# chennachaos/PFEMFort

Measured on AMD Instinct MI355X. Metric: DOF/s (assembly+CG-to-tol), higher is better.
Workload: dtype f64

## Files before the change

### include/pfem_amd_diag.h

```cpp
#ifndef PFEM_AMD_DIAG_H
#define PFEM_AMD_DIAG_H

#include "pfem_amd.h"

#ifdef __cplusplus
extern "C" {
#endif

#define PFEM_ASSEMBLY_GATHER 0
#define PFEM_ASSEMBLY_SCATTER 1
int pfem_solver_set_assembly_mode(pfem_solver *s, int mode);
int pfem_solver_assembly_info(pfem_solver *s, int *gather_form, int *hub_nodes, int *block_threads, int64_t *lds_bytes);
#define PFEM_SPMV_AUTO 0
#define PFEM_SPMV_INT32 1
#define PFEM_SPMV_GAPS16 2
#define PFEM_SPMV_GROUPED 3
int pfem_solver_set_spmv_format(pfem_solver *s, int format);
int pfem_solver_get_spmv_format(pfem_solver *s, int *bits_per_column);
int pfem_solver_get_spmv_row_group(pfem_solver *s, int *rows_per_lane);
int pfem_solver_get_spmv_gap_table(pfem_solver *s, int *entries);
int pfem_solver_get_spmv_value_dictionary(pfem_solver *s, int *entries);
int pfem_solver_amg_value_dictionaries(pfem_solver *s, int max_levels, int *n_levels, int *entries);
int pfem_solver_get_spmv_gap_escapes(pfem_solver *s, int *in_use);
int pfem_solver_spmv_bytes(pfem_solver *s, int64_t *format_bytes);

int pfem_solver_amg_info(pfem_solver *s, int max_levels, int *n_levels, int64_t *rows, int64_t *nnz, double *lambda_max,
                         double *symbolic_ms, double *numeric_ms, int *cheb_degree, int *fine_degree, double *eig_ratio, double *coarse_scale);
int pfem_solver_amg_aggregates(pfem_solver *s, int level, int32_t *agg);
int pfem_solver_amg_transfer(pfem_solver *s, int level, int *rbm, int *fine_bs, int *coarse_bs, int *dim, int64_t *n_nodes, double *node_xyz);
int pfem_solver_amg_layout(pfem_solver *s, int max_levels, int *coupled, int *distributed_levels, int64_t *first_dof, int64_t *local_rows);
int pfem_solver_incidence_patterns(pfem_solver *s, int *count, int *longest);
int pfem_solver_amg_aggregation(pfem_solver *s, int max_levels, int *n_levels, int *kind);
int pfem_solver_amg_comm_counts(pfem_solver *s, int *exchanges_per_cycle, int *allreduces_per_cycle);
int pfem_solver_amg_cycle_profile(pfem_solver *s, int max_levels, int *n_levels, int *exchanges, double *exchange_ms,
                                  int64_t *exchange_doubles, int *allreduces, double *allreduce_ms, int64_t *allreduce_doubles,
                                  double *cycle_ms);
int pfem_solver_amg_pairing(pfem_solver *s, int *lattice_levels);
int pfem_solver_amg_cycle(pfem_solver *s, int *cycle, int *last_level_visited_twice);
int pfem_solver_amg_level0_epilogue(pfem_solver *s, int *taken);

int pfem_eval_elems(pfem_solver *s, const double *elemData, const double *timeData,
                    double *K_out, double *F_out);

int pfem_matrix_info(pfem_solver *s, int64_t *n_owned, int64_t *n_local, int64_t *nnz,
                     int64_t *stored_entries);

int pfem_spmv(pfem_solver *s, const double *x, double *y);
int pfem_bench_spmv(pfem_solver *s, int reps, double *ms_per_launch);

typedef struct pfem_timings {
    double pattern_ms;
    double assemble_ms;
    double solve_ms;
    double spmv_ms_total;
    int64_t spmv_launches;
// ... 28 lines not shown
```

### pfemfort_amd/_lib.py

```python
from __future__ import annotations

import ctypes as C
import os

_HERE = os.path.dirname(os.path.abspath(__file__))
LIB_PATH = os.environ.get("PFEM_AMD_LIB") or os.path.join(_HERE, "libpfem_amd.so")

OK, ERR_ARG, ERR_STATE, ERR_NEG_JAC, ERR_HIP, ERR_NOGPU, ERR_NOMEM, ERR_DIVERGED, ERR_PATTERN, ERR_COMM = range(10)
POISSON_TRIA, POISSON_TET, ELAST_TET, POISSON_TRIA_INLINE, ELAST_TRIA = 1, 2, 3, 4, 5
SOLVER_EMPTY, PATTERN_OK, INIT_OK, ASSEMBLY_OK, FACTORISE_OK = 1, 2, 3, 4, 5
INSERT_VALUES, ADD_VALUES = 1, 2

NPELEM = {POISSON_TRIA: 3, POISSON_TET: 4, ELAST_TET: 4, POISSON_TRIA_INLINE: 3, ELAST_TRIA: 3}
NDOF = {POISSON_TRIA: 1, POISSON_TET: 1, ELAST_TET: 3, POISSON_TRIA_INLINE: 1, ELAST_TRIA: 2}
NDIM = {POISSON_TRIA: 2, POISSON_TET: 3, ELAST_TET: 3, POISSON_TRIA_INLINE: 2, ELAST_TRIA: 2}


class PfemError(RuntimeError):
    def __init__(self, code: int, where: str, detail: str = ""):
        self.code = code
        msg = f"{where}: error {code} ({_strerror(code)})"
        if detail:
            msg += f" -- {detail}"
        super().__init__(msg)
# ... 40 lines not shown
    "pfem_write_vtk": [C.c_char_p, _I, _L, _L, _I, _I, _P, _P, _P, _P],
    "pfem_write_temp_dat": [C.c_char_p, _L, _P, _P, _P],
    "pfem_solver_create": [_P, _L, _L, _L, _P, _P, _I],
    "pfem_solver_destroy": [_P],
    "pfem_solver_set_stream": [_P, _P],
    "pfem_solver_set_tolerances": [_P, _D, _D, _D, _I],
    "pfem_solver_status": [_P, _P],
    "pfem_solver_set_zero": [_P],
    "pfem_solver_print_info": [_P],
    "pfem_mat_set_values": [_P, _I, _P, _I, _P, _P, _I],
    "pfem_vec_set_values": [_P, _I, _P, _P, _I],
    "pfem_solver_assemble_matrix_and_vector": [_P, _I, _P, _P, _P, _P],
    "pfem_solver_factorise": [_P],
    "pfem_solver_solve": [_P, _P, _P, _P],
    "pfem_solver_factorise_and_solve": [_P, _P, _P, _P],
    "pfem_solver_get_solution": [_P, _P],
    "pfem_solver_get_history": [_P, _P, _I, _P],
    "pfem_mesh_upload": [_P, _I, _L, _P, _L, _P, _P, _P],
    "pfem_box_slab_sizes": [_I, _I, _I, _I, _I, _I, _I, _P, _P, _P, _P, _P],
    "pfem_mesh_generate_box": [_P, _I, _D, _D, _I, _D, _D, _I, _D, _D, _I, _I, _I, _I],
    "pfem_box_slab_sizes_axis": [_I, _I, _I, _I, _I, _I, _I, _I, _P, _P, _P, _P, _P, _P, _P, _P],
    "pfem_mesh_generate_box_axis": [_P, _I, _D, _D, _I, _D, _D, _I, _D, _D, _I, _I, _I, _I, _I],
    "pfem_mesh_download": [_P, _P, _P, _P, _P],
    "pfem_pattern_build": [_P],
    "pfem_assemble": [_P, _P, _P],
    "pfem_solver_set_assembly_mode": [_P, _I],
    "pfem_solver_assembly_info": [_P, _P, _P, _P, _P],
    "pfem_solver_set_spmv_format": [_P, _I],
    "pfem_solver_get_spmv_format": [_P, _P],
    "pfem_solver_get_spmv_row_group": [_P, _P],
    "pfem_solver_get_spmv_gap_table": [_P, _P],
    "pfem_solver_get_spmv_value_dictionary": [_P, _P],
    "pfem_solver_amg_value_dictionaries": [_P, _I, _P, _P],
    "pfem_solver_get_spmv_gap_escapes": [_P, _P],
    "pfem_solver_spmv_bytes": [_P, _P],
    "pfem_solver_set_preconditioner": [_P, _I],
    "pfem_solver_get_preconditioner": [_P, _P],
    "pfem_solver_set_cg_single_reduction": [_P, _I],
    "pfem_solver_amg_info": [_P, _I, _P, _P, _P, _P, _P, _P, _P, _P, _P, _P],
    "pfem_solver_amg_aggregates": [_P, _I, _P],
    "pfem_solver_amg_transfer": [_P, _I, _P, _P, _P, _P, _P, _P],
    "pfem_solver_amg_layout": [_P, _I, _P, _P, _P, _P],
    "pfem_solver_amg_aggregation": [_P, _I, _P, _P],
    "pfem_solver_incidence_patterns": [_P, _P, _P],
    "pfem_solver_amg_comm_counts": [_P, _P, _P],
    "pfem_solver_amg_cycle_profile": [_P, _I, _P, _P, _P, _P, _P, _P, _P, _P],
    "pfem_solver_amg_pairing": [_P, _P],
    "pfem_solver_set_amg_options": [_P, _I, _I, _D, _D],
    "pfem_solver_set_amg_cycle": [_P, _I],
    "pfem_solver_amg_cycle": [_P, _P, _P],
    "pfem_solver_amg_level0_epilogue": [_P, _P],
    "pfem_eval_elems": [_P, _P, _P, _P, _P],
    "pfem_rhs_add_values": [_P, _L, _P, _P],
    "pfem_matrix_info": [_P, _P, _P, _P, _P],
    "pfem_get_local_to_global": [_P, _P],
    "pfem_get_csr": [_P, _P, _P, _P],
    "pfem_get_rhs": [_P, _P],
    "pfem_spmv": [_P, _P, _P],
    "pfem_bench_spmv": [_P, _I, _P],
    "pfem_get_timings": [_P, _P],
    "pfem_solver_profile_spmv": [_P, _I],
    "pfem_neighbour_plan": [_I, _I, _P, _P, _P, _P, _P, _P, _P, _P, _P],
    "pfem_solver_set_neighbours": [_P, _I, _P, _P, _P],
    "pfem_rccl_unique_id": [_P],
    "pfem_solver_set_comm_rccl": [_P, _I, _I, _P],
    "pfem_solver_set_comm_host": [_P, _I, _I, HOST_ALLREDUCE_FN, HOST_EXCHANGE_FN, _P],
# ... 61 lines not shown
```

### pfemfort_amd/csrc/pfem_amg.inc

```

constexpr int kAmgMaxLevels = 14;
constexpr int kAmgMatchRounds = 8;
constexpr int kAmgPasses = 3;
constexpr int64_t kAmgReplicateRows = 150000;
constexpr int kAmgRetryBlock = -7701;

inline bool amg_in_effect(const pfem_solver *s)
{
    return s->pc == PFEM_PC_GAMG;
}

inline SellDev amg_sell(const pfem_solver *s, const AmgLevel &L, int64_t rows)
{
    SellDev A;
    if (L.fine) {
        A = s->sell();
    } else {
        A.slice_off = L.slice_off.p;
        A.rowlen = L.rowlen.p;
        A.cols = L.cols.p;
        A.vals = L.vals.p;
    }
    A.n_rows = rows;
    A.n_slices = (rows + 63) / 64;
// ... 2162 lines not shown
                uint64_t last = 0;
                PFEM_HIP(hipMemcpyAsync(&last, ukeys.p + (nnz_c - 1), sizeof(uint64_t), hipMemcpyDeviceToHost, s->stream));
                PFEM_HIP(hipStreamSynchronize(s->stream));
                if (last == ~0ull) --nnz_c;
            }
            L.nnz_c = nnz_c;
            PFEM_TRY(amg_sell_from_keys(s, W, ukeys.p, nnz_c, C));
            PFEM_TRY(L.dst_slot.alloc(static_cast<size_t>(std::max<int64_t>(nnz_c, 1))));
            hipLaunchKernelGGL(k_amg_dst_slots, dim3(grid_for(nnz_c)), dim3(kBlock), 0, s->stream, nnz_c, static_cast<const uint64_t *>(ukeys.p),
                               static_cast<const int64_t *>(C.rowptr.p), static_cast<const int64_t *>(C.slice_off.p), L.dst_slot.p);
            PFEM_TRY(check_kernel("k_amg_dst_slots"));
            PFEM_HIP(hipStreamSynchronize(s->stream));
        }
        phase(l, "Galerkin maps + coarse pattern");
        if (coupled) PFEM_TRY(amg_agree(s, C.stored > INT_MAX ? PFEM_ERR_ARG : PFEM_OK));
        else if (C.stored > INT_MAX) return PFEM_ERR_ARG;
        M.lev.push_back(std::move(Cp));
        {
            AmgLevel &Cn = *M.lev.back();
            amg_galerkin(s, L, Cn, A);
            PFEM_TRY(check_kernel("k_amg_galerkin (symbolic)"));
        }
        n_global = nc_global;
        if (coupled && n_global > kAmgDense && n_global <= static_cast<double>(replicate_rows)) {
            PFEM_TRY(amg_replicate(s, M, W, *M.lev.back(), static_cast<int64_t>(n_global), overlap));
            phase(l, "replicated levels");
            break;
        }
    }
    M.n_last_global = coupled ? static_cast<int64_t>(n_global) : M.lev.back()->n;
    return PFEM_OK;
}

int amg_finish_levels(pfem_solver *s, Amg &M, bool coupled)
{
    for (auto &L : M.lev) PFEM_TRY(amg_alloc_vectors(s, *L));
    AmgLevel &last = *M.lev.back();
    const int64_t n_last = M.n_last_global;
    M.dense = n_last >= 1 && n_last <= kAmgDense && M.lev.size() > 1 && !M.rep;
    if (M.dense) {
        PFEM_TRY(M.dense_inv.alloc(static_cast<size_t>(n_last * n_last)));
        const int bytes = static_cast<int>(n_last * n_last * sizeof(double));
        if (bytes > 65536) {
            PFEM_HIP(hipFuncSetAttribute(reinterpret_cast<const void *>(k_amg_dense_inverse), hipFuncAttributeMaxDynamicSharedMemorySize, bytes));
            PFEM_HIP(hipFuncSetAttribute(reinterpret_cast<const void *>(k_amg_dense_inverse_of), hipFuncAttributeMaxDynamicSharedMemorySize, bytes));
        }
        if (coupled) {
            PFEM_TRY(M.dense_glob.alloc(static_cast<size_t>(n_last * n_last)));
            PFEM_TRY(M.bx_glob.alloc(static_cast<size_t>(2 * kAmgDense)));
            PFEM_TRY(amg_level_gids(s, last));
        }
    }
    if (coupled) PFEM_TRY(M.lam_all.alloc(static_cast<size_t>(std::max<int64_t>(256, 2 * static_cast<int64_t>(M.lev.size()) * s->nranks))));
    M.fused = !coupled && [] { const char *e = std::getenv("PFEM_AMG_FUSED"); return e ? std::atoi(e) != 0 : true; }();
    M.tail_from = -1;
    for (size_t l = 1; l < M.lev.size() && !coupled; ++l)
        if (M.lev[l]->n <= kAmgTailRows && M.lev[l]->nnz <= kAmgTailNnz && M.lev.size() - l <= static_cast<size_t>(kAmgTailLevels)) { M.tail_from = static_cast<int>(l); break; }
    M.w_to = M.tail_from > 0 ? M.tail_from : static_cast<int>(M.lev.size()) - 2;
    M.tail_lds_allowed = 0;
    if (M.tail_from > 0) {
        int64_t rows = 0;
        for (size_t l = static_cast<size_t>(M.tail_from); l < M.lev.size(); ++l) rows += M.lev[l]->n;
        const AmgLevel &T0 = *M.lev[static_cast<size_t>(M.tail_from)];
        const size_t need = static_cast<size_t>(6 * rows) * sizeof(double) + static_cast<size_t>(T0.stored) * 12 + static_cast<size_t>((T0.n + 63) / 64 + 2) * 8;
        if (need > 65536 && need <= 156 * 1024) {
            if (hipFuncSetAttribute(reinterpret_cast<const void *>(k_amg_tail), hipFuncAttributeMaxDynamicSharedMemorySize, static_cast<int>(need)) == hipSuccess)
                M.tail_lds_allowed = need;
            else
                (void)hipGetLastError();
        }
    }
    return PFEM_OK;
}


void amg_knobs(Amg &M)
{
    const char *er = std::getenv("PFEM_AMG_EIG_RATIO"), *cs = std::getenv("PFEM_AMG_COARSE_SCALE");
    M.eig_ratio = er ? std::max(1.5, std::atof(er)) : (M.eig_ratio_given ? M.eig_ratio_opt : M.eig_ratio_auto);
    M.coarse_scale = cs ? std::atof(cs) : (M.coarse_scale_given ? M.coarse_scale_opt : M.coarse_scale_auto);
    if (M.rep) { M.rep->eig_ratio = M.eig_ratio; M.rep->coarse_scale = M.coarse_scale; }
}

int amg_symbolic(pfem_solver *s, bool multi, bool overlap)
{
    if (!s->amg) s->amg.reset(new (std::nothrow) Amg());
    if (!s->amg) return PFEM_ERR_NOMEM;
    Amg &M = *s->amg;
    const auto t0 = std::chrono::steady_clock::now();
    const bool verbose = std::getenv("PFEM_AMG_VERBOSE") != nullptr;
    const size_t malloc_calls0 = dev_pool().st_malloc_calls;
    const size_t malloc_bytes0 = dev_pool().st_malloc;
    const double malloc_ms0 = dev_pool().st_malloc_ms;
    const size_t reused0 = dev_pool().st_reused;
    auto since_t0 = [&](const char *what) {
        if (!verbose) return;
        (void)hipStreamSynchronize(s->stream);
        std::fprintf(stderr, "  gamg symbolic: %-40s at %9.2f ms\n", what, std::chrono::duration<double, std::milli>(std::chrono::steady_clock::now() - t0).count());
    };
    M.coupled = multi && !M.coupled_refused && [] { const char *e = std::getenv("PFEM_AMG_COUPLED"); return e ? std::atoi(e) != 0 : true; }();
    const bool coupled = M.coupled;
    if (const char *e = std::getenv("PFEM_AMG_CHEB_DEGREE")) M.cheb_degree = std::max(1, std::min(6, std::atoi(e)));
    if (const char *e = std::getenv("PFEM_AMG_FINE_DEGREE")) M.fine_degree = std::max(0, std::min(6, std::atoi(e)));
    M.lev.clear();
    M.rep.reset();
// ... 530 lines not shown
        if (L.rbm) {
            PFEM_RBM_DISPATCH(L.bs, L.dim, hipLaunchKernelGGL((k_rbm_prolong<FB, DIM>), dim3(vec_grid(L.n_loc / L.bs)), dim3(kBlock), 0, s->stream, L.n_loc / L.bs,
                static_cast<const int32_t *>(L.node_agg.p), static_cast<const double *>(L.roff.p), L.n_loc / L.bs, static_cast<const double *>(C.x),
                M.coarse_scale, L.x, ctl));
        } else
        hipLaunchKernelGGL(k_amg_prolong, dim3(vec_grid(L.n_loc)), dim3(kBlock), 0, s->stream, L.n_loc, static_cast<const int32_t *>(L.agg.p),
                           static_cast<const double *>(C.x), M.coarse_scale, L.x, ctl);
        if (amg_smooth(s, M, L, b, false, deg_of(l), ctl, false, overlap) != PFEM_OK) return nullptr;
    }
    return M.lev[0]->x;
}

double *amg_apply(pfem_solver *s, Amg &M, const double *r, const CgCtl *ctl, bool first0_done, int last0)
{
    const int nl = static_cast<int>(M.lev.size());
    if (M.lev[0]->fine && s->n_ghost > 0) (void)hipMemsetAsync(M.lev[0]->x + s->n_owned, 0, sizeof(double) * static_cast<size_t>(s->n_ghost), s->stream);
    const bool fuse = M.fused && M.cheb_degree == 2;
    const int tail = (M.fused && M.tail_from > 0) ? M.tail_from : nl;
    auto deg_of = [&](int l) { return (l == 0 && M.fine_degree > 0) ? M.fine_degree : M.cheb_degree; };
    auto fused_level = [&](int l) { return fuse && l >= 1 && l < tail && l < nl - 1; };
    auto ep = [&](int mode, AmgLevel &L, const double *xin, const double *r_in, int step, int add_dd0, double *r_out, double *dd_out, double *x) {
        const SellDev A = amg_sell(s, L);
        const dim3 grid(spmv_grid(A.n_slices)), block(kBlock);
        const double *dinv = L.dinv.p, *lam = L.lam.p;
        if (L.gptr.p && (L.bs == 6 || L.bs == 3)) {
            const int64_t *gp = L.gptr.p;
            const int32_t *gc = L.gcol.p;
#define PFEM_BLK_EP(MODEV, CBV) hipLaunchKernelGGL((k_rbm_spmv_ep<MODEV, CBV>), grid, block, 0, s->stream, A, gp, gc, xin, r_in, dinv, lam, M.eig_ratio, step, add_dd0, r_out, dd_out, x, ctl)
            if (L.bs == 6) { if (mode == kEpNextLast) PFEM_BLK_EP(kEpNextLast, 6); else if (mode == kEpResid) PFEM_BLK_EP(kEpResid, 6); else PFEM_BLK_EP(kEpFirstRes, 6); }
            else { if (mode == kEpNextLast) PFEM_BLK_EP(kEpNextLast, 3); else if (mode == kEpResid) PFEM_BLK_EP(kEpResid, 3); else PFEM_BLK_EP(kEpFirstRes, 3); }
#undef PFEM_BLK_EP
            return;
        }
        if (L.vd_ok && L.vcodes.p) {
            const uint16_t *q = L.vcodes.p;
            const double *d = L.vdict.p;
            const size_t lds = sizeof(double) * static_cast<size_t>(L.vd_n);
            if (mode == kEpNextLast) hipLaunchKernelGGL(k_amg_spmv_ep_vd<kEpNextLast>, grid, block, lds, s->stream, A, q, d, L.vd_n, xin, r_in, dinv, lam, M.eig_ratio, step, add_dd0, r_out, dd_out, x, ctl);
            else if (mode == kEpResid) hipLaunchKernelGGL(k_amg_spmv_ep_vd<kEpResid>, grid, block, lds, s->stream, A, q, d, L.vd_n, xin, r_in, dinv, lam, M.eig_ratio, step, add_dd0, r_out, dd_out, x, ctl);
            else hipLaunchKernelGGL(k_amg_spmv_ep_vd<kEpFirstRes>, grid, block, lds, s->stream, A, q, d, L.vd_n, xin, r_in, dinv, lam, M.eig_ratio, step, add_dd0, r_out, dd_out, x, ctl);
            return;
        }
        if (mode == kEpNextLast) hipLaunchKernelGGL(k_amg_spmv_ep<kEpNextLast>, grid, block, 0, s->stream, A, xin, r_in, dinv, lam, M.eig_ratio, step, add_dd0, r_out, dd_out, x, ctl);
        else if (mode == kEpResid) hipLaunchKernelGGL(k_amg_spmv_ep<kEpResid>, grid, block, 0, s->stream, A, xin, r_in, dinv, lam, M.eig_ratio, step, add_dd0, r_out, dd_out, x, ctl);
        else hipLaunchKernelGGL(k_amg_spmv_ep<kEpFirstRes>, grid, block, 0, s->stream, A, xin, r_in, dinv, lam, M.eig_ratio, step, add_dd0, r_out, dd_out, x, ctl);
    };
    auto run_tail = [&]() {
        AmgTail T{};
        T.nlev = nl - tail;
        T.deg = M.cheb_degree;
        T.coarsest_deg = M.coarsest_sweeps;
        T.dense_n = M.dense ? static_cast<int>(M.lev.back()->n) : 0;
        T.dense_inv = M.dense_inv.p;
        T.ratio = M.eig_ratio;
        T.scale = M.coarse_scale;
        for (int q = 0; q < T.nlev; ++q) {
            AmgLevel &L = *M.lev[static_cast<size_t>(tail + q)];
            AmgTailLevel &t = T.lev[q];
            t.A = amg_sell(s, L);
            t.dinv = L.dinv.p; t.lam = L.lam.p;
            t.x = L.x; t.dd = L.dd; t.t = L.t.p; t.r = L.r.p; t.b = L.b.p;
            t.agg = L.agg.p; t.mem_ptr = L.mem_ptr.p; t.mem_idx = L.mem_idx.p;
            t.n = L.n; t.nc = L.nc; t.stored = L.stored;
            t.rbm_dim = L.rbm ? L.dim : 0; t.fb = L.bs; t.nn = L.n_nodes; t.node_agg = L.node_agg.p; t.roff = L.roff.p;
        }
        int64_t rows = 0;
        for (int q = 0; q < T.nlev; ++q) rows += T.lev[q].n;
        const size_t vec_b = static_cast<size_t>(6 * rows) * sizeof(double);
        const bool use_lds = vec_b <= 65536;
        const AmgTailLevel &t0 = T.lev[0];
        const size_t mat_b = (T.nlev > 1 && t0.stored > 0) ? static_cast<size_t>(t0.stored) * 12 + static_cast<size_t>(t0.A.n_slices + 2) * 8 : 0;
        const bool mat = use_lds && mat_b > 0 && vec_b + mat_b <= 156 * 1024;
        const size_t lds = use_lds ? vec_b + (mat ? mat_b : 0) : 0;
        const bool mat_ok = mat && (lds <= 65536 || lds <= M.tail_lds_allowed);
        hipLaunchKernelGGL(k_amg_tail, dim3(1), dim3(1024), use_lds ? (mat_ok ? lds : vec_b) : 0, s->stream, T, ctl, use_lds ? 1 : 0,
                           mat_ok ? t0.stored : static_cast<int64_t>(0));
    };
    std::function<void(int)> visit = [&](int l) {
// ... 129 lines not shown
    double *sbuf = s->d_sbuf.p;
    CgCtl *ctl = s->d_ctl.p;
    PFEM_TRY(cg_reset_control(s, ctl));
    double host_comm_s = 0.0;
    const int deg0 = M.fine_degree > 0 ? M.fine_degree : M.cheb_degree;
    const bool fuse_first0 = M.fused && M.lev.size() > 1 && !M.coupled;
    const bool fuse_last0 = M.fused && M.lev.size() > 1 && deg0 == 1 && !M.coupled;
    const bool rows4 = !multi && spmv_has_level0_ep(s);
    const bool ep0 = rows4 && fuse_last0;
    const int last0 = ep0 ? kLast0Epilogue : (fuse_last0 ? kLast0Product : kLast0Smooth);
    M.level0_ep = ep0;
    if (rows4 && s->d_part_ep.n < 2 * static_cast<size_t>(gs) + 2 * kFoldBlocks) PFEM_TRY(s->d_part_ep.alloc(2 * static_cast<size_t>(gs) + 2 * kFoldBlocks));
    double *ep_rz = s->d_part_ep.p, *ep_zz = ep_rz ? ep_rz + gs : nullptr, *fold_rz = ep_rz ? ep_zz + gs : nullptr, *fold_zz = ep_rz ? fold_rz + kFoldBlocks : nullptr;
    bool use_vgraph = false;
    {
        const int graph_env = cg_graph_env();
        const bool coupled_capturable = multi && M.coupled && !overlap && s->comm && s->comm->capturable() && s->comm->p2p_capturable() &&
                                        (!M.rep || M.n_last_global <= s->comm->allreduce_capture_limit());
        if ((!multi || coupled_capturable) && graph_env && s->stream != nullptr) {
            std::vector<uint64_t> key = {reinterpret_cast<uint64_t>(s->d_r.p), reinterpret_cast<uint64_t>(ctl), reinterpret_cast<uint64_t>(s->stream),
                                         reinterpret_cast<uint64_t>(s->d_vals.p), reinterpret_cast<uint64_t>(s->d_cols.p), reinterpret_cast<uint64_t>(s->d_rvals.p),
                                         reinterpret_cast<uint64_t>(s->d_gvals.p), reinterpret_cast<uint64_t>(s->d_dwords.p), spmv_key(s),
                                         static_cast<uint64_t>(M.cheb_degree), static_cast<uint64_t>(M.fine_degree), static_cast<uint64_t>(M.dense),
                                         static_cast<uint64_t>(M.eig_ratio * 1e6), static_cast<uint64_t>(M.coarse_scale * 1e6), static_cast<uint64_t>(M.lev.size()),
                                         static_cast<uint64_t>(M.fused), static_cast<uint64_t>(M.tail_from + 1), static_cast<uint64_t>(M.coupled),
                                         static_cast<uint64_t>(M.cycle_gamma), static_cast<uint64_t>(M.w_to + 1),
                                         static_cast<uint64_t>(M.coupled_fused), reinterpret_cast<uint64_t>(s->d_send.p), reinterpret_cast<uint64_t>(s->d_recv.p),
                                         reinterpret_cast<uint64_t>(s->comm), reinterpret_cast<uint64_t>(M.rep.get()), reinterpret_cast<uint64_t>(M.bx_glob.p),
                                         static_cast<uint64_t>(last0), ep0 ? reinterpret_cast<uint64_t>(s->d_part_ep.p) : 0, ep0 ? static_cast<uint64_t>(gs) : 0,
                                         reinterpret_cast<uint64_t>(M.lev[0]->t.p), reinterpret_cast<uint64_t>(M.lev[0]->dinv.p)};
            auto level_key = [&](const std::unique_ptr<AmgLevel> &L) {
                key.push_back(reinterpret_cast<uint64_t>(L->x)); key.push_back(reinterpret_cast<uint64_t>(L->vals.p)); key.push_back(static_cast<uint64_t>(L->n));
                key.push_back(L->vd_ok ? static_cast<uint64_t>(L->vd_n + 1) : 0); key.push_back(reinterpret_cast<uint64_t>(L->vcodes.p));
            };
            for (auto &L : M.lev) level_key(L);
            if (M.rep) for (auto &L : M.rep->lev) level_key(L);
            PFEM_TRY(M.graph.ensure(s->stream, std::move(key), {s->stream}, [&](int) {
                if (M.coupled) return amg_apply_coupled(s, M, s->d_r.p, ctl, overlap) != nullptr;
                (void)amg_apply(s, M, s->d_r.p, ctl, fuse_first0, last0);
                return true;
            }, &use_vgraph));
        }
    }
    auto precondition = [&](const CgCtl *c) -> double * {
        if (use_vgraph && c == ctl) {
            if (hipGraphLaunch(M.graph.exec[0], s->stream) != hipSuccess) return nullptr;
            return ep0 ? M.lev[0]->t.p : M.lev[0]->x;
        }
        if (M.coupled) return amg_apply_coupled(s, M, s->d_r.p, c, overlap);
        double *z = amg_apply(s, M, s->d_r.p, c, c == ctl && fuse_first0, c == ctl ? last0 : kLast0Smooth);
        if (c == ctl && fuse_last0) return z;
        if (multi && exchange_sum(s, z, overlap) != PFEM_OK) return nullptr;
        return z;
    };
    auto dots = [&](double *z, const CgCtl *c, hipEvent_t *cev) -> int {
        if (c == ctl && ep0) return PFEM_OK;
        if (c == ctl && rows4) {
            hipLaunchKernelGGL(k_pc_dots_rows4, dim3(gs), block, 0, s->stream, c, s->n_owned, static_cast<const double *>(s->d_r.p),
                               static_cast<const double *>(z), ep_rz, ep_zz);
            hipLaunchKernelGGL(k_fold_partials2, dim3(kFoldBlocks, 2), block, 0, s->stream, static_cast<const double *>(ep_rz),
                               static_cast<const double *>(ep_zz), static_cast<int>(gs), fold_rz, fold_zz, c);
            return PFEM_OK;
        }
        if (c == ctl && fuse_last0) {
            AmgLevel &L0 = *M.lev[0];
            hipLaunchKernelGGL(k_pc_post_dots, dim3(gv), block, 0, s->stream, c, n, s->n_owned, static_cast<const double *>(s->d_r.p),
// ... 113 lines not shown
```

### pfemfort_amd/csrc/pfem_amg_kernels.hpp

```cpp
#pragma once

namespace pfem {

__device__ __forceinline__ int64_t amg_edge_key(int32_t i, int32_t j, int32_t hi_, int32_t hj_, double w, double di, double dj)
{
    if (!(w < 0.0) || !(di > 0.0) || !(dj > 0.0)) return -1;
    const double s = -w / sqrt(di * dj);
    int b = static_cast<int>(floor(8.0 * log2(s))) + 2048;
    b = b < 1 ? 1 : (b > 4095 ? 4095 : b);
    const int64_t lo = hi_ < hj_ ? hi_ : hj_, hi = hi_ < hj_ ? hj_ : hi_;
    const int64_t close = 0x7fffffffLL - (hi - lo);
    const int64_t par = (lo & 1) == 0;
    const int64_t a = i < j ? i : j, c = i < j ? j : i;
    const int64_t h = ((a * 2654435761LL + c * 40503LL) >> 7) & 0x7ffffLL;
    return (static_cast<int64_t>(b) << 51) | (close << 20) | (par << 19) | h;
}

__global__ void __launch_bounds__(kBlock) k_amg_match_pick(int64_t n, const int64_t *__restrict__ gptr, const int32_t *__restrict__ gcol,
                                                            const double *__restrict__ gw, const double *__restrict__ gdiag,
                                                            const int32_t *__restrict__ hint ,
                                                            const int32_t *__restrict__ match, int32_t *__restrict__ cand)
{
    const int64_t i = static_cast<int64_t>(blockIdx.x) * kBlock + threadIdx.x;
    if (i >= n) return;
// ... 1337 lines not shown
    double acc = 0.0;
    int k = 0;
    for (; k + 4 <= width; k += 4) {
        int c[4];
        uint16_t q[4];
        double xv[4];
#pragma unroll
        for (int j = 0; j < 4; ++j) { c[j] = cp[64 * (k + j)]; q[j] = qp[64 * (k + j)]; }
#pragma unroll
        for (int j = 0; j < 4; ++j) xv[j] = xin[c[j]];
#pragma unroll
        for (int j = 0; j < 4; ++j) acc = __builtin_fma(vd[q[j]], xv[j], acc);
    }
    for (; k < width; ++k) acc = __builtin_fma(vd[qp[64 * k]], xin[cp[64 * k]], acc);
    const int64_t i = (s << 6) + lane;
    if (i >= A.n_rows) return;
    if (MODE == kEpResid) {
        r_out[i] = r_in[i] - acc;
    } else if (MODE == kEpFirstRes) {
        const double ri = r_in[i] - acc;
        r_out[i] = ri;
        dd_out[i] = cheb_coef(lam[0], ratio, 0).c_first * dinv[i] * ri;
    } else {
        const ChebCoef c = cheb_coef(lam[0], ratio, step);
        const double ri = r_in[i] - acc;
        const double d0 = xin[i];
        const double di = __builtin_fma(c.c_dd, d0, c.c_r * dinv[i] * ri);
        double xv = x[i];
        if (add_dd0) xv += d0;
        x[i] = xv + di;
    }
}

__global__ void __launch_bounds__(kBlock) k_amg_spmv_pack(SellDev A, const double *__restrict__ xin, double *__restrict__ y, ShareSum S,
                                                           double *__restrict__ send, const CgCtl *ctl)
{
    if (ctl && ctl->flag != 0) return;
    const int lane = threadIdx.x & 63, wave = threadIdx.x >> 6;
    const int64_t s = (static_cast<int64_t>(blockIdx.x) << 2) + wave;
    if (s >= A.n_slices) return;
    const int64_t off = A.slice_off[s];
    const int width = static_cast<int>((A.slice_off[s + 1] - off) >> 6);
    const int32_t *__restrict__ cp = A.cols + off + lane;
    const double *__restrict__ vp = A.vals + off + lane;
    double acc = 0.0;
    int k = 0;
    for (; k + 4 <= width; k += 4) {
        int c[4];
        double v[4], xv[4];
#pragma unroll
        for (int j = 0; j < 4; ++j) { c[j] = cp[64 * (k + j)]; v[j] = vp[64 * (k + j)]; }
#pragma unroll
        for (int j = 0; j < 4; ++j) xv[j] = xin[c[j]];
#pragma unroll
        for (int j = 0; j < 4; ++j) acc = __builtin_fma(v[j], xv[j], acc);
    }
    for (; k < width; ++k) acc = __builtin_fma(vp[64 * k], xin[cp[64 * k]], acc);
    const int64_t i = (s << 6) + lane;
    if (i >= A.n_rows) return;
    y[i] = acc;
    share_pack(S, send, i, acc);
}

__global__ void __launch_bounds__(kBlock) k_amg_spmv_pack_vd(SellDev A, const uint16_t *__restrict__ codes, const double *__restrict__ dict, int nd,
                                                              const double *__restrict__ xin, double *__restrict__ y, ShareSum S,
                                                              double *__restrict__ send, const CgCtl *ctl)
// ... 457 lines not shown
```

### pfemfort_amd/csrc/pfem_amg_types.hpp

```cpp
#pragma once

struct AmgPlan {
    std::vector<int> peers;
    std::vector<int64_t> peer_off{0};
    std::vector<int32_t> send_lidx;
    int64_t n_send = 0, n_sh = 0;
    DevBuf<int32_t> d_send_lidx, d_sh_lidx, d_sh_ptr, d_sh_src;
    DevBuf<int32_t> d_row_sh;
};

struct AmgLevel {
    int64_t n = 0, n_slices = 0, stored = 0, nnz = 0;
    int64_t n_loc = 0;
    int64_t gid_off = 0;
    std::vector<int64_t> ghost_gid;
    AmgPlan plan;
    DevBuf<int32_t> gid;
    bool fine = false;
    DevBuf<int64_t> slice_off, rowptr;
    DevBuf<int32_t> rowlen, cols;
    DevBuf<double> vals;
    int bs = 1;
    int64_t n_nodes = 0;
    DevBuf<int32_t> node_of, comp_of;
// ... 12 lines not shown
    bool lat_nodes_global = false;
    std::vector<std::pair<int, int>> lat_str[3];
    bool lat_split = false;
    std::vector<double> lat_coord;
    DevBuf<double> xyz;
    int agg_kind = 0;
    int64_t nc = 0;
    DevBuf<int32_t> agg;
    DevBuf<int32_t> mem_ptr, mem_idx;
    int64_t nnz_c = 0;
    DevBuf<int64_t> src_ptr;
    DevBuf<int32_t> src_slot;
    DevBuf<int64_t> dst_slot;
    DevBuf<uint8_t> code_of;
    DevBuf<uint32_t> code_mask;
    int dim = 0;
    bool rbm = false;
    DevBuf<double> cen;
    DevBuf<double> roff;
    DevBuf<int32_t> node_agg;
    DevBuf<int64_t> gptr;
    DevBuf<int32_t> gcol, brow;
    int64_t nblk = 0;
    DevBuf<double> dinv, t, r, b, x_store, dd_store, lam, part_max;
    DevBuf<uint16_t> vcodes;
    DevBuf<double> vdict;
    DevBuf<unsigned long long> vtable;
    int vd_n = 0;
    bool vd_ok = false, vd_have_dict = false, vd_refused = false;
    DevBuf<VdHashEntry> vhash;
    bool vd_hash_ok = false;
    bool vd_direct = false;
    bool bound_fresh = false;
    double *x = nullptr, *dd = nullptr;
    DevBuf<double> x1;
    double lam_host = 0.0;
};

struct Amg {
    std::vector<std::unique_ptr<AmgLevel>> lev;
    DevBuf<double> dense_inv;
    bool dense = false;
    bool symbolic_ok = false;
    bool galerkin_fresh = false;
    double symbolic_ms = 0.0, numeric_ms = 0.0;
    int cheb_degree = 2;
    int fine_degree = 1;
    bool eig_ratio_given = false;
    bool coarse_scale_given = false;
    double eig_ratio_opt = 0.0, coarse_scale_opt = 0.0;
    double eig_ratio_auto = 16.0, coarse_scale_auto = 1.5;
    double eig_ratio = 8.0, coarse_scale = 1.5;
    CgGraph graph;
    hipEvent_t ev_num0 = nullptr, ev_num1 = nullptr;
    ~Amg()
    {
        if (ev_num0) (void)hipEventDestroy(ev_num0);
        if (ev_num1) (void)hipEventDestroy(ev_num1);
    }
    int tail_from = -1;
    size_t tail_lds_allowed = 0;
    int cycle_gamma = 1, w_to = -1;
    bool cycle_given = false;
    bool fused = true;
    bool level0_ep = false;
    int coarsest_sweeps = 8;
// ... 15 lines not shown
```

### pfemfort_amd/csrc/pfem_device.hip

```cpp
#include <hip/hip_runtime.h>
#include <hip/hip_ext.h>
#include <hipcub/hipcub.hpp>
#include <rccl/rccl.h>
#include <dlfcn.h>

#include <algorithm>
#include <chrono>
#include <climits>
#include <cmath>
#include <cstdio>
#include <cstdlib>
#include <cstring>
#include <mutex>
#include <thread>
#include <string>
#include <deque>
#include <functional>
#include <map>
#include <memory>
#include <vector>

#include "pfem_internal.hpp"
#include "pfem_vdhash.hpp"
#include "pfem_kernels.hpp"
// ... 4670 lines not shown
    (void)hipEventDestroy(c0);
    (void)hipEventDestroy(c1);
    PFEM_TRY(rc);
    return s->comm->health();
}

extern "C" int pfem_solver_set_amg_options(pfem_solver *s, int cheb_degree, int fine_degree, double eig_ratio, double coarse_scale)
{
    if (!s || cheb_degree < 1 || cheb_degree > 6 || fine_degree < 0 || fine_degree > 6 || (eig_ratio > 0.0 && !(eig_ratio > 1.0))) return PFEM_ERR_ARG;
    if (!s->amg) s->amg.reset(new (std::nothrow) Amg());
    if (!s->amg) return PFEM_ERR_NOMEM;
    s->amg->cheb_degree = cheb_degree;
    s->amg->fine_degree = fine_degree;
    s->amg->graph.invalidate();
    s->amg->eig_ratio_given = eig_ratio > 0.0;
    if (eig_ratio > 0.0) s->amg->eig_ratio_opt = eig_ratio;
    s->amg->coarse_scale_given = coarse_scale > 0.0;
    if (coarse_scale > 0.0) s->amg->coarse_scale_opt = coarse_scale;
    return PFEM_OK;
}

extern "C" int pfem_solver_amg_value_dictionaries(pfem_solver *s, int max_levels, int *n_levels, int *entries)
{
    if (!s || !n_levels || !entries || max_levels < 1) return PFEM_ERR_ARG;
    *n_levels = 0;
    if (!s->amg || !s->amg->symbolic_ok) return PFEM_OK;
    for (const AmgLevelRef &r : amg_levels_of(*s->amg)) {
        if (*n_levels >= max_levels) break;
        entries[(*n_levels)++] = r.L->fine ? ((s->vd_ok && s->vd_current) ? s->vd_n : 0) : (r.L->vd_ok ? r.L->vd_n : 0);
    }
    return PFEM_OK;
}

extern "C" int pfem_solver_set_amg_cycle(pfem_solver *s, int cycle)
{
    if (!s || cycle < 0 || cycle > 2) return PFEM_ERR_ARG;
    if (!s->amg) s->amg.reset(new (std::nothrow) Amg());
    if (!s->amg) return PFEM_ERR_NOMEM;
    s->amg->cycle_given = cycle != 0;
    if (cycle != 0) s->amg->cycle_gamma = cycle;
    s->amg->graph.invalidate();
    return PFEM_OK;
}
extern "C" int pfem_solver_amg_level0_epilogue(pfem_solver *s, int *taken)
{
    if (!s || !taken) return PFEM_ERR_ARG;
    if (!s->amg || !s->amg->symbolic_ok) return PFEM_ERR_STATE;
    *taken = s->amg->level0_ep ? 1 : 0;
    return PFEM_OK;
}

extern "C" int pfem_solver_amg_cycle(pfem_solver *s, int *cycle, int *last_level_visited_twice)
{
    if (!s || !cycle || !last_level_visited_twice) return PFEM_ERR_ARG;
    if (!s->amg || !s->amg->symbolic_ok) return PFEM_ERR_STATE;
    const Amg &M = *s->amg;
    *cycle = M.cycle_gamma;
    *last_level_visited_twice = M.cycle_gamma > 1 ? std::min(M.w_to, static_cast<int>(M.lev.size()) - 2) : 0;
    return PFEM_OK;
}
```

### pfemfort_amd/solver.py

```python
from __future__ import annotations

import ctypes as C

import numpy as np

from . import _lib as L
from ._lib import (ADD_VALUES, ASSEMBLY_OK, FACTORISE_OK, INIT_OK, INSERT_VALUES,
                   PATTERN_OK, SOLVER_EMPTY)


def _p(a):
    return None if a is None else a.ctypes.data_as(C.c_void_p)


def _f64(a):
    return np.ascontiguousarray(a, dtype=np.float64)


def _i32(a):
    return np.ascontiguousarray(a, dtype=np.int32)


class PetscSolver:

# ... 131 lines not shown
        L.check(L.lib().pfem_pattern_build(self._h), "pfem_pattern_build")

    def setAssemblyMode(self, mode):
        L.check(L.lib().pfem_solver_set_assembly_mode(self._h, {"gather": 0, "scatter": 1}[mode]),
                "pfem_solver_set_assembly_mode")

    def assemblyInfo(self):
        g = C.c_int(0); h = C.c_int(0); t = C.c_int(0); b = C.c_int64(0)
        L.check(L.lib().pfem_solver_assembly_info(self._h, C.byref(g), C.byref(h), C.byref(t), C.byref(b)), "pfem_solver_assembly_info")
        return {"gather": bool(g.value), "hub_nodes": h.value, "block_threads": t.value, "lds_bytes": b.value}

    def setSpmvFormat(self, fmt):
        L.check(L.lib().pfem_solver_set_spmv_format(self._h, {"auto": 0, "int32": 1, "gaps16": 2, "grouped": 3}[fmt]), "pfem_solver_set_spmv_format")

    def spmvColumnBits(self):
        b = C.c_int(0)
        L.check(L.lib().pfem_solver_get_spmv_format(self._h, C.byref(b)), "pfem_solver_get_spmv_format")
        return b.value

    def spmvGapTable(self):
        b = C.c_int(0)
        L.check(L.lib().pfem_solver_get_spmv_gap_table(self._h, C.byref(b)), "pfem_solver_get_spmv_gap_table")
        return b.value

    def spmvValueDictionary(self):
        b = C.c_int(0)
        L.check(L.lib().pfem_solver_get_spmv_value_dictionary(self._h, C.byref(b)), "pfem_solver_get_spmv_value_dictionary")
        return b.value

    def amgValueDictionaries(self):
        n = C.c_int(0)
        e = (C.c_int * 32)()
        L.check(L.lib().pfem_solver_amg_value_dictionaries(self._h, 32, C.byref(n), e), "pfem_solver_amg_value_dictionaries")
        return list(e[:n.value])

    def spmvGapEscapes(self):
        b = C.c_int(0)
        L.check(L.lib().pfem_solver_get_spmv_gap_escapes(self._h, C.byref(b)), "pfem_solver_get_spmv_gap_escapes")
        return bool(b.value)

    def setPreconditioner(self, pc):
        L.check(L.lib().pfem_solver_set_preconditioner(self._h, {"jacobi": 0, "pbjacobi": 1, "gamg": 2}[pc]), "pfem_solver_set_preconditioner")

    def setSingleReduction(self, on=True):
        L.check(L.lib().pfem_solver_set_cg_single_reduction(self._h, -1 if on is None else int(bool(on))),
                "pfem_solver_set_cg_single_reduction")

    def preconditioner(self):
        b = C.c_int(0)
        L.check(L.lib().pfem_solver_get_preconditioner(self._h, C.byref(b)), "pfem_solver_get_preconditioner")
        return ("jacobi", "pbjacobi", "gamg")[b.value]

    def setAmgOptions(self, cheb_degree=2, fine_degree=1, eig_ratio=None, coarse_scale=None):
        L.check(L.lib().pfem_solver_set_amg_options(self._h, cheb_degree, fine_degree, -1.0 if eig_ratio is None else eig_ratio,
                                                    -1.0 if coarse_scale is None else coarse_scale), "pfem_solver_set_amg_options")

    def setAmgCycle(self, cycle=None):
        code = {None: 0, "auto": 0, "v": 1, "w": 2}[cycle.lower() if isinstance(cycle, str) else cycle]
        L.check(L.lib().pfem_solver_set_amg_cycle(self._h, code), "pfem_solver_set_amg_cycle")

    def amgCycle(self):
        c, w, e = C.c_int(0), C.c_int(0), C.c_int(0)
        L.check(L.lib().pfem_solver_amg_cycle(self._h, C.byref(c), C.byref(w)), "pfem_solver_amg_cycle")
        L.check(L.lib().pfem_solver_amg_level0_epilogue(self._h, C.byref(e)), "pfem_solver_amg_level0_epilogue")
        return {"cycle": "w" if c.value == 2 else "v", "last_level_visited_twice": w.value, "level0_epilogue": bool(e.value)}

# ... 190 lines not shown
```

Before: 617.7 million.

## Compress AMG coarse-level column indices to byte offsets in fused smoother SpMV

On the intermediate AMG levels (scalar, single rank, fused path), the distinct column-minus-row offsets are collected into a device hash table. When there are at most 256 of them, each int32 column index is replaced by an 8-bit code into a sorted offset table held in LDS, and four codes are packed per word. The fused Chebyshev/residual SpMV becomes a single templated deep-batched kernel that reads these packed codes, combined with the value dictionary when it is available, and prefetches batches of 16 entries. This is meant to cut index bandwidth on the coarse levels. In exchange it adds setup work with host syncs and extra LDS lookups and decode arithmetic in the inner loop.

```diff
diff --git a/include/pfem_amd_diag.h b/include/pfem_amd_diag.h
--- a/include/pfem_amd_diag.h
+++ b/include/pfem_amd_diag.h
@@ -21,6 +21,7 @@
 int pfem_solver_get_spmv_gap_table(pfem_solver *s, int *entries);
 int pfem_solver_get_spmv_value_dictionary(pfem_solver *s, int *entries);
 int pfem_solver_amg_value_dictionaries(pfem_solver *s, int max_levels, int *n_levels, int *entries);
+int pfem_solver_amg_column_forms(pfem_solver *s, int max_levels, int *n_levels, int *entries);
 int pfem_solver_get_spmv_gap_escapes(pfem_solver *s, int *in_use);
 int pfem_solver_spmv_bytes(pfem_solver *s, int64_t *format_bytes);
 
diff --git a/pfemfort_amd/_lib.py b/pfemfort_amd/_lib.py
--- a/pfemfort_amd/_lib.py
+++ b/pfemfort_amd/_lib.py
@@ -96,6 +96,7 @@
     "pfem_solver_get_spmv_gap_table": [_P, _P],
     "pfem_solver_get_spmv_value_dictionary": [_P, _P],
     "pfem_solver_amg_value_dictionaries": [_P, _I, _P, _P],
+    "pfem_solver_amg_column_forms": [_P, _I, _P, _P],
     "pfem_solver_get_spmv_gap_escapes": [_P, _P],
     "pfem_solver_spmv_bytes": [_P, _P],
     "pfem_solver_set_preconditioner": [_P, _I],
diff --git a/pfemfort_amd/csrc/pfem_amg.inc b/pfemfort_amd/csrc/pfem_amg.inc
--- a/pfemfort_amd/csrc/pfem_amg.inc
+++ b/pfemfort_amd/csrc/pfem_amg.inc
@@ -2218,6 +2218,53 @@
     return PFEM_OK;
 }
 
+int amg_column_offsets(pfem_solver *s, Amg &M)
+{
+    const int nl = static_cast<int>(M.lev.size());
+    for (auto &L : M.lev) { L->coff_n = 0; L->coff.release(); L->cidx.release(); L->cidx_off.release(); }
+    if (!M.fused || M.coupled || s->nranks > 1) return PFEM_OK;
+    const int tail = M.tail_from > 0 ? M.tail_from : nl;
+    DevBuf<int32_t> table;
+    DevBuf<int> meta;
+    DevBuf<int64_t> words;
+    DevBuf<char> temp;
+    for (int l = 1; l < tail && l < nl - 1; ++l) {
+        AmgLevel &L = *M.lev[static_cast<size_t>(l)];
+        if (L.fine || L.bs != 1 || L.gptr.p || L.n < 1 || L.n >= (1LL << 30)) continue;
+        const SellDev A = amg_sell(s, L);
+        if (!table.p) { PFEM_TRY(table.alloc(kCoffTable)); PFEM_TRY(meta.alloc(2)); }
+        PFEM_HIP(hipMemsetAsync(table.p, 0x80, sizeof(int32_t) * kCoffTable, s->stream));
+        PFEM_HIP(hipMemsetAsync(meta.p, 0, 2 * sizeof(int), s->stream));
+        PFEM_TRY(L.coff.alloc(kCoffMax));
+        hipLaunchKernelGGL(k_coff_collect, dim3(spmv_grid(A.n_slices)), dim3(kBlock), 0, s->stream, A, table.p, meta.p);
+        hipLaunchKernelGGL(k_coff_finish, dim3(1), dim3(kCoffTable), 0, s->stream, static_cast<const int32_t *>(table.p), L.coff.p, meta.p);
+        PFEM_TRY(check_kernel("k_coff_collect / k_coff_finish"));
+        int m[2] = {0, 0};
+        PFEM_HIP(hipMemcpyAsync(m, meta.p, sizeof m, hipMemcpyDeviceToHost, s->stream));
+        PFEM_HIP(hipStreamSynchronize(s->stream));
+        if (m[0] < 1 || m[0] > kCoffMax) {
+            L.coff.release();
+            if (std::getenv("PFEM_AMG_VERBOSE")) std::fprintf(stderr, "  level %d: more than %d distinct column offsets, the fused products keep the int32 columns\n", l, kCoffMax);
+            continue;
+        }
+        PFEM_TRY(words.reserve(static_cast<size_t>(A.n_slices) + 1));
+        PFEM_TRY(L.cidx_off.alloc(static_cast<size_t>(A.n_slices) + 1));
+        hipLaunchKernelGGL(k_cidx_sizes, dim3(grid_for(A.n_slices + 1)), dim3(kBlock), 0, s->stream, A.n_slices, A.slice_off, words.p);
+        PFEM_TRY(amg_exclusive_sum(s, temp, static_cast<const int64_t *>(words.p), L.cidx_off.p, A.n_slices + 1));
+        int64_t total = 0;
+        PFEM_HIP(hipMemcpyAsync(&total, L.cidx_off.p + A.n_slices, sizeof(int64_t), hipMemcpyDeviceToHost, s->stream));
+        PFEM_HIP(hipStreamSynchronize(s->stream));
+        PFEM_TRY(L.cidx.alloc(static_cast<size_t>(std::max<int64_t>(total, 1))));
+        hipLaunchKernelGGL(k_cidx_fill, dim3(spmv_grid(A.n_slices)), dim3(kBlock), 0, s->stream, A, static_cast<const int32_t *>(L.coff.p), m[0], m[1],
+                           static_cast<const int64_t *>(L.cidx_off.p), L.cidx.p);
+        PFEM_TRY(check_kernel("k_cidx_fill"));
+        L.coff_n = m[0];
+        L.coff_zero = m[1];
+    }
+    PFEM_HIP(hipStreamSynchronize(s->stream));
+    return PFEM_OK;
+}
+
 int amg_finish_levels(pfem_solver *s, Amg &M, bool coupled)
 {
     for (auto &L : M.lev) PFEM_TRY(amg_alloc_vectors(s, *L));
@@ -2256,7 +2303,7 @@
                 (void)hipGetLastError();
         }
     }
-    return PFEM_OK;
+    return amg_column_offsets(s, M);
 }
 
 
@@ -2853,18 +2900,22 @@
 #undef PFEM_BLK_EP
             return;
         }
-        if (L.vd_ok && L.vcodes.p) {
-            const uint16_t *q = L.vcodes.p;
-            const double *d = L.vdict.p;
-            const size_t lds = sizeof(double) * static_cast<size_t>(L.vd_n);
-            if (mode == kEpNextLast) hipLaunchKernelGGL(k_amg_spmv_ep_vd<kEpNextLast>, grid, block, lds, s->stream, A, q, d, L.vd_n, xin, r_in, dinv, lam, M.eig_ratio, step, add_dd0, r_out, dd_out, x, ctl);
-            else if (mode == kEpResid) hipLaunchKernelGGL(k_amg_spmv_ep_vd<kEpResid>, grid, block, lds, s->stream, A, q, d, L.vd_n, xin, r_in, dinv, lam, M.eig_ratio, step, add_dd0, r_out, dd_out, x, ctl);
-            else hipLaunchKernelGGL(k_amg_spmv_ep_vd<kEpFirstRes>, grid, block, lds, s->stream, A, q, d, L.vd_n, xin, r_in, dinv, lam, M.eig_ratio, step, add_dd0, r_out, dd_out, x, ctl);
-            return;
-        }
-        if (mode == kEpNextLast) hipLaunchKernelGGL(k_amg_spmv_ep<kEpNextLast>, grid, block, 0, s->stream, A, xin, r_in, dinv, lam, M.eig_ratio, step, add_dd0, r_out, dd_out, x, ctl);
-        else if (mode == kEpResid) hipLaunchKernelGGL(k_amg_spmv_ep<kEpResid>, grid, block, 0, s->stream, A, xin, r_in, dinv, lam, M.eig_ratio, step, add_dd0, r_out, dd_out, x, ctl);
-        else hipLaunchKernelGGL(k_amg_spmv_ep<kEpFirstRes>, grid, block, 0, s->stream, A, xin, r_in, dinv, lam, M.eig_ratio, step, add_dd0, r_out, dd_out, x, ctl);
+        const bool vd = L.vd_ok && L.vcodes.p, offs = L.coff_n > 0 && L.cidx.p;
+        const uint32_t *ci = L.cidx.p;
+        const int64_t *cio = L.cidx_off.p;
+        const int32_t *co = L.coff.p;
+        const uint16_t *q = L.vcodes.p;
+        const double *d = L.vdict.p;
+        const int nd = vd ? L.vd_n : 0;
+        const size_t lds = sizeof(double) * static_cast<size_t>(nd) + (offs ? sizeof(int32_t) * kCoffMax : 0);
+#define PFEM_EP_DEEP(MODEV, VDV, OFFSV) hipLaunchKernelGGL((k_amg_spmv_ep_deep<MODEV, VDV, OFFSV>), grid, block, lds, s->stream, A, ci, cio, co, L.coff_n, q, d, nd, xin, r_in, dinv, lam, M.eig_ratio, step, add_dd0, r_out, dd_out, x, ctl)
+#define PFEM_EP_MODE(VDV, OFFSV) do { if (mode == kEpNextLast) PFEM_EP_DEEP(kEpNextLast, VDV, OFFSV); else if (mode == kEpResid) PFEM_EP_DEEP(kEpResid, VDV, OFFSV); else PFEM_EP_DEEP(kEpFirstRes, VDV, OFFSV); } while (0)
+        if (vd && offs) PFEM_EP_MODE(true, true);
+        else if (vd) PFEM_EP_MODE(true, false);
+        else if (offs) PFEM_EP_MODE(false, true);
+        else PFEM_EP_MODE(false, false);
+#undef PFEM_EP_MODE
+#undef PFEM_EP_DEEP
     };
     auto run_tail = [&]() {
         AmgTail T{};
@@ -3060,6 +3111,8 @@
             auto level_key = [&](const std::unique_ptr<AmgLevel> &L) {
                 key.push_back(reinterpret_cast<uint64_t>(L->x)); key.push_back(reinterpret_cast<uint64_t>(L->vals.p)); key.push_back(static_cast<uint64_t>(L->n));
                 key.push_back(L->vd_ok ? static_cast<uint64_t>(L->vd_n + 1) : 0); key.push_back(reinterpret_cast<uint64_t>(L->vcodes.p));
+                key.push_back(static_cast<uint64_t>(L->coff_n)); key.push_back(reinterpret_cast<uint64_t>(L->cidx.p));
+                key.push_back(reinterpret_cast<uint64_t>(L->cidx_off.p)); key.push_back(reinterpret_cast<uint64_t>(L->coff.p));
             };
             for (auto &L : M.lev) level_key(L);
             if (M.rep) for (auto &L : M.rep->lev) level_key(L);
diff --git a/pfemfort_amd/csrc/pfem_amg_kernels.hpp b/pfemfort_amd/csrc/pfem_amg_kernels.hpp
--- a/pfemfort_amd/csrc/pfem_amg_kernels.hpp
+++ b/pfemfort_amd/csrc/pfem_amg_kernels.hpp
@@ -1393,6 +1393,176 @@
     }
 }
 
+constexpr int kCoffMax = 256;
+constexpr int kCoffTable = 1024;
+constexpr int32_t kCoffEmpty = static_cast<int32_t>(0x80808080u);
+__device__ __forceinline__ void coff_insert(int32_t d, int32_t *table, int *meta)
+{
+    unsigned h = (static_cast<uint32_t>(d) * 2654435761u) >> 22;
+    for (int probe = 0; probe < kCoffTable; ++probe, h = (h + 1) & (kCoffTable - 1)) {
+        int32_t cur = __hip_atomic_load(table + h, __ATOMIC_RELAXED, __HIP_MEMORY_SCOPE_AGENT);
+        if (cur == d) return;
+        if (cur != kCoffEmpty) continue;
+        cur = atomicCAS(table + h, kCoffEmpty, d);
+        if (cur == d) return;
+        if (cur == kCoffEmpty) { atomicAdd(meta, 1); return; }
+    }
+    atomicAdd(meta, kCoffMax + 1);
+}
+__global__ void __launch_bounds__(kBlock) k_coff_collect(SellDev A, int32_t *table, int *meta)
+{
+    const int lane = threadIdx.x & 63, wave = threadIdx.x >> 6;
+    const int64_t s = (static_cast<int64_t>(blockIdx.x) << 2) + wave;
+    if (s >= A.n_slices) return;
+    const int64_t i = (s << 6) + lane;
+    if (i >= A.n_rows) return;
+    const int64_t off = A.slice_off[s];
+    const int width = static_cast<int>((A.slice_off[s + 1] - off) >> 6);
+    const int32_t *__restrict__ cp = A.cols + off + lane;
+    coff_insert(0, table, meta);
+    for (int k = 0; k < width; ++k) {
+        if (__hip_atomic_load(meta, __ATOMIC_RELAXED, __HIP_MEMORY_SCOPE_AGENT) > kCoffMax) return;
+        coff_insert(cp[64 * k] - static_cast<int32_t>(i), table, meta);
+    }
+}
+__global__ void __launch_bounds__(kCoffTable) k_coff_finish(const int32_t *__restrict__ table, int32_t *__restrict__ coff, int *meta)
+{
+    __shared__ int32_t v[kCoffTable];
+    const int32_t mine = table[threadIdx.x];
+    v[threadIdx.x] = mine;
+    __syncthreads();
+    if (meta[0] > kCoffMax || mine == kCoffEmpty) return;
+    int rank = 0;
+    for (int u = 0; u < kCoffTable; ++u) rank += (v[u] != kCoffEmpty && v[u] < mine) ? 1 : 0;
+    coff[rank] = mine;
+    if (mine == 0) meta[1] = rank;
+}
+__global__ void __launch_bounds__(kBlock) k_cidx_sizes(int64_t n_slices, const int64_t *__restrict__ slice_off, int64_t *__restrict__ words)
+{
+    const int64_t s = static_cast<int64_t>(blockIdx.x) * kBlock + threadIdx.x;
+    if (s > n_slices) return;
+    words[s] = s < n_slices ? 64 * ((((slice_off[s + 1] - slice_off[s]) >> 6) + 3) >> 2) : 0;
+}
+__global__ void __launch_bounds__(kBlock) k_cidx_fill(SellDev A, const int32_t *__restrict__ coff, int nco, int zero_idx,
+                                                       const int64_t *__restrict__ cidx_off, uint32_t *__restrict__ cidx)
+{
+    __shared__ int32_t co[kCoffMax];
+    for (int i = threadIdx.x; i < nco; i += kBlock) co[i] = coff[i];
+    __syncthreads();
+    const int lane = threadIdx.x & 63, wave = threadIdx.x >> 6;
+    const int64_t s = (static_cast<int64_t>(blockIdx.x) << 2) + wave;
+    if (s >= A.n_slices) return;
+    const int64_t i = (s << 6) + lane;
+    const int64_t off = A.slice_off[s];
+    const int width = static_cast<int>((A.slice_off[s + 1] - off) >> 6);
+    const int32_t *__restrict__ cp = A.cols + off + lane;
+    uint32_t *__restrict__ ip = cidx + cidx_off[s] + lane;
+    for (int j = 0; 4 * j < width; ++j) {
+        uint32_t w = 0;
+        for (int b = 0; b < 4; ++b) {
+            const int k = 4 * j + b;
+            int idx = zero_idx;
+            if (k < width && i < A.n_rows) {
+                const int32_t d = cp[64 * k] - static_cast<int32_t>(i);
+                int lo = 0, hi = nco - 1;
+                while (lo < hi) { const int mid = (lo + hi) >> 1; if (co[mid] < d) lo = mid + 1; else hi = mid; }
+                idx = lo;
+            }
+            w |= static_cast<uint32_t>(idx) << (8 * b);
+        }
+        ip[64 * j] = w;
+    }
+}
+
+constexpr int kEpBatch = 16;
+template <int MODE, bool VD, bool OFFS>
+__global__ void __launch_bounds__(kBlock) k_amg_spmv_ep_deep(SellDev A, const uint32_t *__restrict__ cidx, const int64_t *__restrict__ cidx_off,
+                                                              const int32_t *__restrict__ coff, int nco, const uint16_t *__restrict__ codes,
+                                                              const double *__restrict__ dict, int nd, const double *__restrict__ xin,
+                                                              const double *r_in, const double *__restrict__ dinv, const double *__restrict__ lam,
+                                                              double ratio, int step, int add_dd0, double *r_out, double *dd_out, double *x,
+                                                              const CgCtl *ctl)
+{
+    extern __shared__ double vd[];
+    constexpr int NG = kEpBatch / 4;
+    if (ctl && ctl->flag != 0) return;
+    const int lane = threadIdx.x & 63, wave = __builtin_amdgcn_readfirstlane(threadIdx.x >> 6);
+    const int64_t s = (static_cast<int64_t>(blockIdx.x) << 2) + wave;
+    const bool live = s < A.n_slices;
+    int64_t off = 0, ioff = 0;
+    int width = 0;
+    if (live) {
+        off = A.slice_off[s];
+        width = static_cast<int>((A.slice_off[s + 1] - off) >> 6);
+        if (OFFS) ioff = cidx_off[s];
+    }
+    const uint32_t *__restrict__ ip = cidx + ioff + lane;
+    const int32_t *__restrict__ cp = A.cols + off + lane;
+    const uint16_t *__restrict__ qp = codes + off + lane;
+    const double *__restrict__ vp = A.vals + off + lane;
+    const int64_t i = (s << 6) + lane;
+    const int32_t rowb = i < A.n_rows ? static_cast<int32_t>(i) : 0;
+    uint32_t w[NG];
+    int c[kEpBatch];
+    uint16_t q[kEpBatch];
+    double v[kEpBatch], xv[kEpBatch];
+#define PFEM_EP_STREAM(K0)                                                                          \
+    _Pragma("unroll") for (int g = 0; g < NG; ++g)                                                  \
+        if ((K0) + 4 * g < width) {                                                                 \
+            if (OFFS) w[g] = ip[64 * (((K0) >> 2) + g)];                                            \
+            _Pragma("unroll") for (int j = 0; j < 4; ++j) {                                         \
+                const int kk = min((K0) + 4 * g + j, width - 1);                                    \
+                if (!OFFS) c[4 * g + j] = cp[64 * kk];                                              \
+                if (VD) q[4 * g + j] = qp[64 * kk]; else v[4 * g + j] = vp[64 * kk];                \
+            }                                                                                       \
+        }
+    PFEM_EP_STREAM(0)
+    int32_t *co = reinterpret_cast<int32_t *>(vd + (VD ? nd : 0));
+    if (VD) for (int t = threadIdx.x; t < nd; t += kBlock) vd[t] = dict[t];
+    if (OFFS) for (int t = threadIdx.x; t < nco; t += kBlock) co[t] = coff[t];
+    if (VD || OFFS) __syncthreads();
+    if (!live) return;
+    double acc = 0.0;
+    for (int k0 = 0;;) {
+#pragma unroll
+        for (int g = 0; g < NG; ++g)
+            if (k0 + 4 * g < width) {
+#pragma unroll
+                for (int j = 0; j < 4; ++j) {
+                    const int col = OFFS ? rowb + co[(w[g] >> (8 * j)) & 255u] : c[4 * g + j];
+                    xv[4 * g + j] = xin[col];
+                }
+            }
+#pragma unroll
+        for (int g = 0; g < NG; ++g)
+            if (k0 + 4 * g < width) {
+#pragma unroll
+                for (int j = 0; j < 4; ++j)
+                    if (k0 + 4 * g + j < width) acc = __builtin_fma(VD ? vd[q[4 * g + j]] : v[4 * g + j], xv[4 * g + j], acc);
+            }
+        k0 += kEpBatch;
+        if (k0 >= width) break;
+        PFEM_EP_STREAM(k0)
+    }
+#undef PFEM_EP_STREAM
+    if (i >= A.n_rows) return;
+    if (MODE == kEpResid) {
+        r_out[i] = r_in[i] - acc;
+    } else if (MODE == kEpFirstRes) {
+        const double ri = r_in[i] - acc;
+        r_out[i] = ri;
+        dd_out[i] = cheb_coef(lam[0], ratio, 0).c_first * dinv[i] * ri;
+    } else {
+        const ChebCoef c = cheb_coef(lam[0], ratio, step);
+        const double ri = r_in[i] - acc;
+        const double d0 = xin[i];
+        const double di = __builtin_fma(c.c_dd, d0, c.c_r * dinv[i] * ri);
+        double xv = x[i];
+        if (add_dd0) xv += d0;
+        x[i] = xv + di;
+    }
+}
+
 __global__ void __launch_bounds__(kBlock) k_amg_spmv_pack(SellDev A, const double *__restrict__ xin, double *__restrict__ y, ShareSum S,
                                                            double *__restrict__ send, const CgCtl *ctl)
 {
diff --git a/pfemfort_amd/csrc/pfem_amg_types.hpp b/pfemfort_amd/csrc/pfem_amg_types.hpp
--- a/pfemfort_amd/csrc/pfem_amg_types.hpp
+++ b/pfemfort_amd/csrc/pfem_amg_types.hpp
@@ -68,6 +68,10 @@
     bool vd_hash_ok = false;
     bool vd_direct = false;
     bool bound_fresh = false;
+    DevBuf<int32_t> coff;
+    DevBuf<uint32_t> cidx;
+    DevBuf<int64_t> cidx_off;
+    int coff_n = 0, coff_zero = 0;
     double *x = nullptr, *dd = nullptr;
     DevBuf<double> x1;
     double lam_host = 0.0;
diff --git a/pfemfort_amd/csrc/pfem_device.hip b/pfemfort_amd/csrc/pfem_device.hip
--- a/pfemfort_amd/csrc/pfem_device.hip
+++ b/pfemfort_amd/csrc/pfem_device.hip
@@ -4726,6 +4726,18 @@
     return PFEM_OK;
 }
 
+extern "C" int pfem_solver_amg_column_forms(pfem_solver *s, int max_levels, int *n_levels, int *entries)
+{
+    if (!s || !n_levels || !entries || max_levels < 1) return PFEM_ERR_ARG;
+    *n_levels = 0;
+    if (!s->amg || !s->amg->symbolic_ok) return PFEM_OK;
+    for (const AmgLevelRef &r : amg_levels_of(*s->amg)) {
+        if (*n_levels >= max_levels) break;
+        entries[(*n_levels)++] = (!r.L->fine && r.L->cidx.p) ? r.L->coff_n : 0;
+    }
+    return PFEM_OK;
+}
+
 extern "C" int pfem_solver_set_amg_cycle(pfem_solver *s, int cycle)
 {
     if (!s || cycle < 0 || cycle > 2) return PFEM_ERR_ARG;
diff --git a/pfemfort_amd/solver.py b/pfemfort_amd/solver.py
--- a/pfemfort_amd/solver.py
+++ b/pfemfort_amd/solver.py
@@ -187,6 +187,12 @@
         n = C.c_int(0)
         e = (C.c_int * 32)()
         L.check(L.lib().pfem_solver_amg_value_dictionaries(self._h, 32, C.byref(n), e), "pfem_solver_amg_value_dictionaries")
+        return list(e[:n.value])
+
+    def amgColumnForms(self):
+        n = C.c_int(0)
+        e = (C.c_int * 32)()
+        L.check(L.lib().pfem_solver_amg_column_forms(self._h, 32, C.byref(n), e), "pfem_solver_amg_column_forms")
         return list(e[:n.value])
 
     def spmvGapEscapes(self):
```

Result: slower. 609.5 million (-1.3%).
